# aptx4869lm/4DCapture-FPV

Hardware: AMD Instinct MI355X
Metric: frames/sec global-opt (fixed iters), 1024f clip/500k-pt scene; Chamfer GB/s (higher is better)
Workload: dtype f32; 1 GPU; BASELINE config 3: 1024-frame clip, 500000-pt scene, 500 contact verts, 500 Adam iterations (phase split 0.8), full loss; frames sharded over 1 GPU(s); frames=1024, scene_points=500000, contact_verts=500, iters=500, body_verts=10475, lbs_weights_per_vertex=4

## Files before the change

### 4dcapture-fpv_amd/capi.py

```python
from __future__ import annotations

import ctypes
import os
from ctypes import POINTER, c_char_p, c_double, c_float, c_int32, c_int64, c_void_p

import numpy as np

_HERE = os.path.dirname(os.path.abspath(__file__))
LIB_PATH = os.environ.get("FDCAP_LIB") or os.path.join(_HERE, "libfdcap_hip.so")

NUM_LOSSES = 8
XDIM = 78
PDIM = 75


class FdcapError(RuntimeError):
    pass


class ModelDesc(ctypes.Structure):
    _fields_ = [("num_verts", c_int32), ("v_template", POINTER(c_float)), ("shapedirs", POINTER(c_float)),
                ("num_shape", c_int32), ("posedirs", POINTER(c_float)), ("J_regressor", POINTER(c_float)),
                ("parents", POINTER(c_int32)), ("lbs_weights", POINTER(c_float)),
                ("hands_componentsl", POINTER(c_float)), ("hands_componentsr", POINTER(c_float)),
# ... 26 lines not shown
    "fdcap_ctx_create": (c_int32, [POINTER(ModelDesc), POINTER(c_void_p)]),
    "fdcap_ctx_destroy": (None, [c_void_p]),
    "fdcap_set_scene": (c_int32, [c_void_p, c_void_p, c_int64]),
    "fdcap_debug_scene_hash": (c_int32, [c_void_p, c_void_p]),
    "fdcap_debug_scene_table": (c_int32, [c_void_p, c_int32, c_void_p, POINTER(c_int64)]),
    "fdcap_debug_kernel_forms": (c_int32, [c_void_p, c_int32, c_int32]),
    "fdcap_set_contact_ids": (c_int32, [c_void_p, c_void_p, c_int32]),
    "fdcap_chamfer_fwd": (c_int32, [c_void_p, c_void_p, c_void_p, c_int32, c_int32, c_int32, c_int64, c_void_p,
                                     c_void_p, c_void_p, c_void_p, c_void_p]),
    "fdcap_chamfer_bwd": (c_int32, [c_void_p, c_void_p, c_void_p, c_int32, c_int32, c_int32, c_int64, c_void_p,
                                     c_void_p, c_void_p, c_void_p]),
    "fdcap_chamfer_fwd_scene": (c_int32, [c_void_p, c_void_p, c_int32, c_int32, c_void_p, c_void_p, c_int32, c_void_p]),
    "fdcap_chamfer_bwd_scene": (c_int32, [c_void_p, c_void_p, c_int32, c_int32, c_void_p, c_void_p, c_void_p, c_void_p]),
    "fdcap_set_nn_kernel": (c_int32, [c_int32]),
    "fdcap_vposer_decode": (c_int32, [c_void_p, c_void_p, c_int32, c_int32, c_void_p, c_void_p, c_void_p]),
    "fdcap_vposer_decode_bwd": (c_int32, [c_void_p, c_void_p, c_int32, c_int32, c_void_p, c_void_p, c_void_p, c_void_p]),
    "fdcap_smplx_backward": (c_int32, [c_void_p] * 7 + [c_int32] + [c_void_p] * 9),
    "fdcap_body_forward": (c_int32, [c_void_p, c_void_p, c_int32, c_void_p, c_void_p, c_void_p]),
    "fdcap_world_mesh": (c_int32, [c_void_p, c_void_p, c_int32, c_void_p, c_void_p, c_void_p, c_void_p]),
    "fdcap_params_75_to_78": (c_int32, [c_void_p, c_int32, c_void_p, c_void_p]),
    "fdcap_params_78_to_75": (c_int32, [c_void_p, c_int32, c_void_p, c_void_p]),
    "fdcap_smplx_forward": (c_int32, [c_void_p, c_void_p, c_void_p, c_void_p, c_void_p, c_void_p, c_void_p, c_int32,
                                       c_void_p, c_void_p, c_void_p]),
    "fdcap_opt_create": (c_int32, [c_void_p, POINTER(OptConfig), c_void_p, c_void_p, c_void_p, c_void_p, c_void_p]),
    "fdcap_opt_create_clips": (c_int32, [c_void_p, POINTER(OptConfig), c_int32, c_void_p, c_void_p, c_void_p, c_void_p, c_void_p]),
    "fdcap_opt_set_inputs": (c_int32, [c_void_p, c_void_p, c_void_p, c_void_p, c_void_p, c_void_p]),
    "fdcap_opt_backward": (c_int32, [c_void_p, c_int32, c_int32, c_int32, c_void_p]),
    "fdcap_opt_step": (c_int32, [c_void_p, c_int32, c_int32, c_void_p]),
    "fdcap_opt_backward_and_step": (c_int32, [c_void_p, c_int32, c_int32, c_int32, c_void_p]),
    "fdcap_opt_sync": (c_int32, [c_void_p, c_void_p]),
    "fdcap_opt_run": (c_int32, [c_void_p, c_int32, c_int32, c_int32, c_int32, c_int32, c_void_p, c_int32, c_int32, c_void_p, c_void_p]),
    "fdcap_comm_unique_id": (c_int32, [c_void_p]),
    "fdcap_comm_create": (c_int32, [c_void_p, c_void_p, c_int32, c_int32]),
    "fdcap_comm_destroy": (c_int32, [c_void_p]),
    "fdcap_comm_last_error": (c_char_p, [c_void_p]),
    "fdcap_opt_halo_exchange": (c_int32, [c_void_p, c_void_p]),
    "fdcap_opt_exchange": (c_int32, [c_void_p, c_int32, c_int32, c_void_p]),
    "fdcap_opt_time_exchange": (c_int32, [c_void_p, c_int32, POINTER(c_float), POINTER(c_float), c_void_p]),
    "fdcap_comm_allreduce_f64": (c_int32, [c_void_p, c_void_p, c_int32, c_void_p]),
    "fdcap_opt_state_len": (c_int32, [c_void_p]),
    "fdcap_opt_export_state": (c_int32, [c_void_p, c_void_p, c_void_p]),
    "fdcap_opt_import_state": (c_int32, [c_void_p, c_void_p, c_void_p]),
    "fdcap_opt_check_finite": (c_int32, [c_void_p, c_void_p, c_void_p]),
    "fdcap_opt_set_loss_output": (c_int32, [c_void_p, c_void_p]),
    "fdcap_opt_detect_contact": (c_int32, [c_void_p, c_int32, c_void_p, c_void_p]),
    "fdcap_opt_backward_local2": (c_int32, [c_void_p, c_void_p, c_int32, c_void_p]),
    "fdcap_opt_step_x": (c_int32, [c_void_p, c_int32, c_void_p]),
    "fdcap_opt_set_dct": (c_int32, [c_void_p, c_void_p, c_int32, c_int32, c_void_p, c_void_p]),
    "fdcap_opt_dct_fit": (c_int32, [c_void_p, c_int32, c_int32, c_float, c_void_p, c_int32, c_void_p]),
    "fdcap_opt_backward_dct": (c_int32, [c_void_p, c_float, c_float, c_float, c_int32, c_void_p]),
    "fdcap_opt_set_dct_coef": (c_int32, [c_void_p, c_void_p, c_void_p]),
    "fdcap_opt_get_dct": (c_int32, [c_void_p, c_void_p, c_void_p]),
    "fdcap_opt_get_dct_state": (c_int32, [c_void_p, c_void_p, c_void_p, c_void_p]),
    "fdcap_opt_set_dct_state": (c_int32, [c_void_p, c_void_p, c_void_p, c_void_p]),
    "fdcap_opt_dct_windows": (c_int32, [c_void_p, POINTER(c_int32), POINTER(c_int32)]),
    "fdcap_frame_smoother": (c_int32, [c_void_p, c_void_p, c_int32, c_int32, c_float, c_float, c_float, c_float,
                                        c_void_p, c_int32, c_int32, c_void_p, c_void_p]),
    "fdcap_opt_set_keypoints": (c_int32, [c_void_p, c_void_p, c_void_p]),
    "fdcap_opt_backward_fit2d": (c_int32, [c_void_p, POINTER(Fit2dStage), c_int32, c_void_p]),
    "fdcap_opt_reset_adam": (c_int32, [c_void_p, c_void_p]),
    "fdcap_lbfgs_create": (c_int32, [c_int32, POINTER(LbfgsConfig), POINTER(c_void_p)]),
    "fdcap_lbfgs_destroy": (None, [c_void_p]),
    "fdcap_lbfgs_reset": (c_int32, [c_void_p, c_void_p]),
    "fdcap_lbfgs_advance": (c_int32, [c_void_p, c_void_p, c_int32, c_void_p, c_void_p, c_int32, c_void_p, c_void_p]),
    "fdcap_lbfgs_get_stats": (c_int32, [c_void_p, c_void_p, c_void_p, c_void_p, c_void_p]),
    "fdcap_lbfgs_finalize": (c_int32, [c_void_p, c_void_p, c_int32, c_void_p, c_void_p]),
    "fdcap_opt_fit2d_lbfgs": (c_int32, [c_void_p, POINTER(Fit2dStage), POINTER(LbfgsConfig), c_int32, POINTER(c_int32), c_void_p]),
    "fdcap_opt_fit2d_lbfgs_stats": (c_int32, [c_void_p, c_void_p, c_void_p, c_void_p, c_void_p]),
    "fdcap_opt_step_rows_and_pack": (c_int32, [c_void_p, c_int32, c_int32, c_void_p, c_void_p]),
    "fdcap_opt_unpack_and_step_scale": (c_int32, [c_void_p, c_int32, c_int32, c_void_p, c_int32, c_int32, c_void_p]),
    "fdcap_opt_forward_ahead": (c_int32, [c_void_p, c_int32, c_int32, c_int32, c_void_p]),
    "fdcap_exchange_len": (c_int32, []),
    "fdcap_opt_get_results": (c_int32, [c_void_p, c_void_p, c_void_p, c_void_p, c_void_p]),
    "fdcap_opt_destroy": (None, [c_void_p]),
    "fdcap_opt_forward_world": (c_int32, [c_void_p, c_void_p, c_void_p, c_void_p]),
    "fdcap_opt_get_contact": (c_int32, [c_void_p, c_void_p, c_void_p, c_void_p]),
    "fdcap_opt_get_grads": (c_int32, [c_void_p, c_void_p, c_void_p, c_void_p]),
    "fdcap_panel_gemm": (c_int32, [c_void_p, c_int32, c_int32, c_int32, c_void_p, c_int64, c_int64, c_int32, c_void_p, c_int32,
                                   c_void_p]),
    "fdcap_time_blend_gemm": (c_int32, [c_void_p, c_int32, c_int32, POINTER(c_float), c_void_p]),
    "fdcap_opt_nn_timing": (c_int32, [c_void_p, c_int32]),
    "fdcap_opt_nn_timing_read": (c_int32, [c_void_p, POINTER(c_float), POINTER(c_int32)]),
    "fdcap_debug_nn_query_order": (c_int32, [c_void_p, c_int32, c_void_p, c_int32]),
    "fdcap_opt_launch_timing": (c_int32, [c_void_p, c_int32]),
    "fdcap_opt_launch_timing_read": (c_int32, [c_void_p, c_void_p, c_void_p]),
    "fdcap_opt_time_chamfer": (c_int32, [c_void_p, c_int32, c_int32, POINTER(c_float), c_void_p]),
}

_lib = None


def load_library(path: str | None = None) -> ctypes.CDLL:
    global _lib
    if _lib is not None and path is None:
        return _lib
    p = path or LIB_PATH
    if not os.path.exists(p):
        raise FdcapError(f"{p} is missing: build it with `python -c 'import __graft_entry__ as g; g.build()'` "
                         "(hipcc --offload-arch=gfx950).  There is no CPU fallback.")
    lib = ctypes.CDLL(p)
    for name, (res, args) in SYMBOLS.items():
        fn = getattr(lib, name)
        fn.restype = res
        fn.argtypes = args
    info = lib.fdcap_build_info().decode()
    if "packed_fp32=off" not in info and os.environ.get("FDCAP_ALLOW_PK_F32") != "1":
        raise FdcapError(f"{p} was built with packed fp32 instructions ({info}): results are not reliable next to another kernel's "
                         "MFMAs on the same CU (NOTES.md section 6).  Rebuild with __graft_entry__.build(), or set "
                         "FDCAP_ALLOW_PK_F32=1 for an instrumentation variant.")
    if path is None:
        _lib = lib
    return lib


def count_packed_fp32(path: str | None = None) -> int:
    import re
    import shutil
    import subprocess
    import tempfile
    objdump = os.environ.get("LLVM_OBJDUMP", "/opt/rocm/lib/llvm/bin/llvm-objdump")
    if not os.path.exists(objdump):
        raise FdcapError(f"{objdump} not found (set LLVM_OBJDUMP)")
    with tempfile.TemporaryDirectory() as tmp:
        so = os.path.join(tmp, "lib.so")
        shutil.copy(path or LIB_PATH, so)
        subprocess.run([objdump, "--offloading", so], check=True, capture_output=True, cwd=tmp)
        objs = [f for f in os.listdir(tmp) if "amdgcn" in f]
        if not objs:
            raise FdcapError("no gfx950 code object found in the library")
        n = 0
        for f in objs:
            txt = subprocess.run([objdump, "-d", os.path.join(tmp, f)], check=True, capture_output=True, text=True).stdout
            n += len(re.findall(r"\bv_pk_(?:fma|mul|add)_f32\b", txt))
        return n


def check(code: int, what: str) -> None:
    if code == 0:
        return
    if code < 0:
        names = {-1: "FDCAP_E_ARG", -2: "FDCAP_E_STATE", -3: "FDCAP_E_NODEVICE", -4: "FDCAP_E_COMM (RCCL)"}
        raise FdcapError(f"{what}: {names.get(code, code)}")
    raise FdcapError(f"{what}: hipError_t {code}")


def _f32(a):
    return np.ascontiguousarray(a, dtype=np.float32)


def _fp(a):
    return a.ctypes.data_as(POINTER(c_float))


def dptr(t):
    if t is None:
        return None
    if not t.is_cuda:
        raise FdcapError("expected a device tensor (the HIP path has no host fallback)")
    if not t.is_contiguous():
        raise FdcapError("expected a contiguous tensor")
    return c_void_p(t.data_ptr())


def current_stream():
    import torch
    return c_void_p(torch.cuda.current_stream().cuda_stream)
# ... 57 lines not shown
```

### 4dcapture-fpv_amd/csrc/fdc_api_opt.h

```cpp
#pragma once

extern "C" {

void fdcap_opt_destroy(fdcap_ctx* c) {
    if (!c || !c->opt) return;
    OptState* o = c->opt;
    DevBuf<float>* fb[] = {&o->X0, &o->mask, &o->mX, &o->vX, &o->mCAM, &o->vCAM, &o->mS, &o->vS,
                           &o->H1, &o->H2, &o->O, &o->dO, &o->Opart, &o->dZpart, &o->Rm, &o->PF, &o->Jrest, &o->G, &o->A, &o->M,
                           &o->Jw, &o->Voff, &o->Vw, &o->dist, &o->pd, &o->dVoff, &o->dA, &o->dtransl_v, &o->dMv,
                           &o->dsv, &o->dPF, &o->dJw, &o->dX, &o->dCAM, &o->dscale_row, &o->loss_rows, &o->VoffF, &o->VwF, &o->dVF};
    for (auto* b : fb) b->release();
    o->dctD.release(); o->dctCoef.release(); o->dctM.release(); o->dctV.release(); o->adam_tab.release();
    o->idx.release(); o->pi.release(); o->seedpt.release(); o->kp2d.release(); o->floss.release();
    if (o->lbfgs) { fdcap_lbfgs_destroy(o->lbfgs); o->lbfgs = nullptr; }
    o->nnc_ids.release(); o->nnc_hdr.release(); o->nnc_anchor.release();
    for (hipEvent_t e : o->nn_ev) (void)hipEventDestroy(e);
    o->nn_ev.clear();
    for (hipEvent_t e : o->lt.ev) (void)hipEventDestroy(e);
    o->lt.ev.clear(); o->lt.what.clear(); o->lt.on = false; o->lt.used = 0;
    delete o;
    c->opt = nullptr;
}

static_assert(LROW == FDCAP_NUM_LOSSES, "a batch's per-clip loss slots are LROW apart on the device");
// ... 263 lines not shown

int fdcap_opt_set_loss_output(fdcap_ctx* c, double* losses_d) {
    if (!c || !c->opt || !losses_d) return FDCAP_E_ARG;
    c->opt->log_pending = false;
    c->opt->log_dst = nullptr;
    c->opt->losses.p = losses_d;
    return FDCAP_OK;
}

int fdcap_opt_forward_ahead(fdcap_ctx* c, int32_t ii, int32_t P, int32_t log_terms, void* stream) {
    if (!c || !c->opt || c->opt->nclip > 1) return FDCAP_E_STATE;
    { int es_ = opt_sync(c, (hipStream_t)stream); if (es_) return es_; }
    OptState* o = c->opt;
    hipStream_t st = (hipStream_t)stream;
    const int nl = o->cfg.n_local, nc = c->nc;
    int e = opt_pose_forward(c, 2, 2 + nl, st);
    if (e) return e;
    const bool contact_fwd = o->contact_on && ((ii < P && o->cfg.phase1_contact != 0.f) || log_terms);
    if (contact_fwd) HIP_TRY(blend_forward(c->contact, o->PF.p + 2 * NPFX, nl, o->Voff.p + (size_t)2 * nc * 3, st));
    o->ahead = true;
    o->ahead_blend = contact_fwd;
    return (int)hipGetLastError();
}

int fdcap_opt_backward(fdcap_ctx* c, int32_t ii, int32_t P, int32_t log_terms, void* stream) {
    if (!c || !c->opt) return FDCAP_E_STATE;
    const fdcap_opt_config& cf = c->opt->cfg;
    const bool phase2 = ii >= P;
    LossWeights lw;
    lw.rec = 1.f;
    lw.smooth = phase2 ? cf.phase2_smooth : cf.phase1_smooth;
    lw.contact = phase2 ? 0.f : cf.phase1_contact;
    lw.world = phase2 ? cf.phase2_world : 0.f;
    lw.dct = 0.f;
    lw.world_on = phase2;
    return opt_backward_impl(c, lw, log_terms, (hipStream_t)stream);
}

int fdcap_opt_backward_and_step(fdcap_ctx* c, int32_t ii, int32_t P, int32_t log_terms, void* stream) {
    if (!c || !c->opt) return FDCAP_E_STATE;
    OptState* o = c->opt;
    const fdcap_opt_config& cf = o->cfg;
    const bool fuse = opt_whole_clips(o) && o->dctW == 0;
    if (!fuse) {
        const int e = fdcap_opt_backward(c, ii, P, log_terms, stream);
        return e ? e : fdcap_opt_step(c, ii, P, stream);
    }
    const bool phase2 = ii >= P;
    LossWeights lw;
    lw.rec = 1.f;
    lw.smooth = phase2 ? cf.phase2_smooth : cf.phase1_smooth;
    lw.contact = phase2 ? 0.f : cf.phase1_contact;
    lw.world = phase2 ? cf.phase2_world : 0.f;
    lw.dct = 0.f;
    lw.world_on = phase2;
    return opt_backward_impl(c, lw, log_terms, (hipStream_t)stream, ii, P);
}

int fdcap_debug_nn_query_order(fdcap_ctx* c, int32_t mode, const int32_t* perm_host, int32_t n) {
    if (!c || !c->opt) return FDCAP_E_STATE;
    if (mode < 0 || mode > 2) return FDCAP_E_ARG;
    OptState* o = c->opt;
    NNOrder& ord = o->nn_order;
    if (!o->contact_on || ord.qbuf == nullptr) return FDCAP_E_STATE;
    const int nq = o->cfg.n_local * c->nc;
    if (mode == 2) {
        if (!perm_host || n != nq) return FDCAP_E_ARG;
        std::vector<char> seen((size_t)nq, 0);
        for (int i = 0; i < nq; ++i) {
            if (perm_host[i] < 0 || perm_host[i] >= nq || seen[perm_host[i]]) return FDCAP_E_ARG;
            seen[perm_host[i]] = 1;
        }
    }
    HIP_TRY(hipDeviceSynchronize());
    if (mode == 2) HIP_TRY(hipMemcpy(ord.qbuf, perm_host, (size_t)nq * sizeof(int), hipMemcpyHostToDevice));
    HIP_TRY(hipMemset(o->nnc_hdr.p, 0xFF, (size_t)(nq + 31) / 32 * sizeof(int)));
    ord.perm_mode = mode;
    ord.perm_n = mode == 2 ? nq : 0;
    ord.sorted_groups = 0;
    ord.age = 0;
    return FDCAP_OK;
}

}
```

### 4dcapture-fpv_amd/csrc/fdc_scene.h

```cpp
#pragma once
#include <hip/hip_runtime.h>

#include <algorithm>
#include <utility>
#include <vector>

#include "fdc_chamfer.h"

namespace fdc {

constexpr int SC_RS_ROUNDS = 16;
constexpr int SC_RS_TILE = 256 * SC_RS_ROUNDS;
constexpr int SC_SCAN_BATCH = 16;
constexpr int SC_PT_TILE = 1024;
constexpr int SC_SUPER = 16;

__device__ __forceinline__ unsigned sc_key(float v) {
    unsigned u = __float_as_uint(v);
    if ((u << 1) == 0u) u = 0u;
    return (u & 0x80000000u) ? ~u : (u | 0x80000000u);
}

__global__ __launch_bounds__(256) void sc_keys_kernel(const float* __restrict__ xyz, int n, int axis, unsigned* __restrict__ keys,
                                                      int* __restrict__ vals) {
    const int i = blockIdx.x * 256 + threadIdx.x;
    if (i < n) { keys[i] = sc_key(xyz[3 * (size_t)i + axis]); vals[i] = i; }
}

__global__ __launch_bounds__(256) void sc_rs_hist_kernel(const unsigned* __restrict__ keys, int n, int shift, unsigned* __restrict__ hist, int nb) {
    __shared__ unsigned h[256];
    h[threadIdx.x] = 0;
    __syncthreads();
    const int base = blockIdx.x * SC_RS_TILE;
    for (int r = 0; r < SC_RS_ROUNDS; ++r) {
        const int i = base + r * 256 + threadIdx.x;
        if (i < n) atomicAdd(&h[(keys[i] >> shift) & 255u], 1u);
    }
    __syncthreads();
    hist[(size_t)threadIdx.x * nb + blockIdx.x] = h[threadIdx.x];
}

__global__ __launch_bounds__(1024) void sc_scan_kernel(unsigned* __restrict__ a, int m) {
    __shared__ unsigned part[1024];
    a += (size_t)blockIdx.x * m;
    const int per = (m + 1023) / 1024;
    const int lo = min(m, (int)threadIdx.x * per), hi = min(m, lo + per);
    unsigned s = 0;
    for (int i0 = lo; i0 < hi; i0 += SC_SCAN_BATCH) {
        unsigned v[SC_SCAN_BATCH];
#pragma unroll
        for (int k = 0; k < SC_SCAN_BATCH; ++k) v[k] = i0 + k < hi ? a[i0 + k] : 0u;
#pragma unroll
        for (int k = 0; k < SC_SCAN_BATCH; ++k) s += v[k];
    }
    part[threadIdx.x] = s;
    __syncthreads();
    for (int o = 1; o < 1024; o <<= 1) {
        unsigned t = threadIdx.x >= (unsigned)o ? part[threadIdx.x - o] : 0u;
        __syncthreads();
        part[threadIdx.x] += t;
        __syncthreads();
    }
    unsigned run = part[threadIdx.x] - s;
    for (int i0 = lo; i0 < hi; i0 += SC_SCAN_BATCH) {
        unsigned v[SC_SCAN_BATCH];
#pragma unroll
        for (int k = 0; k < SC_SCAN_BATCH; ++k) v[k] = i0 + k < hi ? a[i0 + k] : 0u;
#pragma unroll
        for (int k = 0; k < SC_SCAN_BATCH; ++k)
            if (i0 + k < hi) { a[i0 + k] = run; run += v[k]; }
    }
}

__global__ __launch_bounds__(256) void sc_rs_scatter_kernel(const unsigned* __restrict__ kin, const int* __restrict__ vin,
                                                            unsigned* __restrict__ kout, int* __restrict__ vout, int n, int shift,
                                                            const unsigned* __restrict__ hist, int nb) {
    __shared__ unsigned base[256];
    __shared__ unsigned wcnt[4][256];
    const int tid = threadIdx.x, wave = tid >> 6, lane = tid & 63;
    base[tid] = hist[(size_t)tid * nb + blockIdx.x];
    const int tile0 = blockIdx.x * SC_RS_TILE;
    for (int r = 0; r < SC_RS_ROUNDS; ++r) {
        const int i = tile0 + r * 256 + tid;
        const bool valid = i < n;
        const unsigned key = valid ? kin[i] : 0u;
        const int val = valid ? vin[i] : 0;
        const unsigned d = (key >> shift) & 255u;
        unsigned long long m = __ballot(valid);
#pragma unroll
        for (int b = 0; b < 8; ++b) {
            const bool bit = (d >> b) & 1u;
            const unsigned long long bal = __ballot(bit);
            m &= bit ? bal : ~bal;
        }
        const int rank = __popcll(m & ((1ull << lane) - 1ull));
        for (int k = 0; k < 4; ++k) wcnt[k][tid] = 0;
        __syncthreads();
        if (valid && rank == 0) wcnt[wave][d] = (unsigned)__popcll(m);
        __syncthreads();
        if (valid) {
            unsigned off = base[d];
            for (int k = 0; k < wave; ++k) off += wcnt[k][d];
            kout[off + rank] = key;
            vout[off + rank] = val;
        }
        __syncthreads();
        base[tid] += wcnt[0][tid] + wcnt[1][tid] + wcnt[2][tid] + wcnt[3][tid];
        __syncthreads();
    }
}

static inline size_t nn_query_order_ints(int nq) { return 4 * (size_t)nq + 256 * (size_t)((nq + SC_RS_TILE - 1) / SC_RS_TILE); }

__global__ __launch_bounds__(256) void nn_order_keys_kernel(const float4* __restrict__ seedpt, int nq, unsigned* __restrict__ key,
                                                            int* __restrict__ val, int* __restrict__ hdr, int groups) {
    const int i = blockIdx.x * 256 + threadIdx.x;
    if (i < nq) {
        const int pos = __float_as_int(seedpt[i].w);
        key[i] = pos >= 0 ? min((unsigned)pos >> 7, 0xFFFFu) : 0xFFFFu;
        val[i] = i;
    }
    if (i < groups) hdr[i] = -1;
}

static inline hipError_t nn_query_order(const float4* seedpt, int nq, int* qbuf, int* hdr, int groups, hipStream_t st) {
    const int nb = (nq + SC_RS_TILE - 1) / SC_RS_TILE;
    int* const perm = qbuf;
    int* const val = qbuf + nq;
    unsigned* const key = (unsigned*)(qbuf + 2 * (size_t)nq);
    unsigned* const hist = key + 2 * (size_t)nq;
    hipLaunchKernelGGL(nn_order_keys_kernel, dim3((std::max(nq, groups) + 255) / 256), dim3(256), 0, st, seedpt, nq, key, perm, hdr, groups);
    for (int pass = 0; pass < 2; ++pass) {
        unsigned* const kin = key + (size_t)pass * nq;
        unsigned* const kout = key + (size_t)(1 - pass) * nq;
        hipLaunchKernelGGL(sc_rs_hist_kernel, dim3(nb), dim3(256), 0, st, kin, nq, 8 * pass, hist, nb);
        hipLaunchKernelGGL(sc_scan_kernel, dim3(1), dim3(1024), 0, st, hist, 256 * nb);
        hipLaunchKernelGGL(sc_rs_scatter_kernel, dim3(nb), dim3(256), 0, st, kin, pass ? val : perm, kout, pass ? perm : val, nq, 8 * pass, hist, nb);
    }
    return hipGetLastError();
}

__device__ __forceinline__ int sc_find_node(const int4* __restrict__ nodes, int nn, int p) {
    int lo = 0, hi = nn - 1;
    while (lo < hi) {
        const int mid = (lo + hi + 1) >> 1;
        if (nodes[mid].x <= p) lo = mid; else hi = mid - 1;
    }
    return lo;
}

__global__ __launch_bounds__(256) void sc_axis_kernel(const int4* __restrict__ nodes, int nn, const float* __restrict__ xyz,
                                                      const int* __restrict__ Lx, const int* __restrict__ Ly, const int* __restrict__ Lz,
                                                      unsigned char* __restrict__ axis) {
    const int i = blockIdx.x * 256 + threadIdx.x;
    if (i >= nn) return;
    const int4 nd = nodes[i];
    int ax = 0;
    if (nd.z < nd.y) {
        const int a = nd.x, b = nd.x + nd.y - 1;
        const float ex = xyz[3 * (size_t)Lx[b]] - xyz[3 * (size_t)Lx[a]];
        const float ey = xyz[3 * (size_t)Ly[b] + 1] - xyz[3 * (size_t)Ly[a] + 1];
        const float ez = xyz[3 * (size_t)Lz[b] + 2] - xyz[3 * (size_t)Lz[a] + 2];
        float best = ex;
        if (ey > best) { ax = 1; best = ey; }
        if (ez > best) { ax = 2; }
    }
    axis[i] = (unsigned char)ax;
}

__global__ __launch_bounds__(256) void sc_side_kernel(const int4* __restrict__ nodes, int nn, const unsigned char* __restrict__ axis,
                                                      const int* __restrict__ Lx, const int* __restrict__ Ly, const int* __restrict__ Lz,
                                                      int n, unsigned char* __restrict__ side) {
    const int p = blockIdx.x * 256 + threadIdx.x;
    if (p >= n) return;
    const int nd = sc_find_node(nodes, nn, p);
    const int4 d = nodes[nd];
    const int ax = axis[nd];
    const int id = (ax == 0 ? Lx : ax == 1 ? Ly : Lz)[p];
    side[id] = (unsigned char)((p - d.x) >= d.z);
}

struct ScLists { const int* in[4]; int* out[4]; };

__device__ __forceinline__ int sc_wave_incl_scan(int v) {
    const int lane = threadIdx.x & 63;
#pragma unroll
    for (int o = 1; o < 64; o <<= 1) { const int t = __shfl_up(v, o); if (lane >= o) v += t; }
    return v;
}

__global__ __launch_bounds__(256) void sc_part_count_kernel(ScLists L, const unsigned char* __restrict__ side, int n, unsigned* __restrict__ cnt, int nb) {
    __shared__ unsigned tot[4];
    if (threadIdx.x < 4) tot[threadIdx.x] = 0;
    __syncthreads();
    const int p0 = blockIdx.x * SC_PT_TILE + threadIdx.x * 4;
    for (int l = 0; l < 4; ++l) {
        int c = 0;
        for (int k = 0; k < 4; ++k) if (p0 + k < n) c += side[L.in[l][p0 + k]];
        const int s = sc_wave_incl_scan(c);
        if ((threadIdx.x & 63) == 63) atomicAdd(&tot[l], (unsigned)s);
    }
    __syncthreads();
    if (threadIdx.x < 4) cnt[(size_t)threadIdx.x * nb + blockIdx.x] = tot[threadIdx.x];
}

__global__ __launch_bounds__(256) void sc_part_scatter_kernel(ScLists L, const unsigned char* __restrict__ side, int n,
                                                              const int4* __restrict__ nodes, int nn, const unsigned* __restrict__ cnt, int nb) {
    __shared__ int wsum[4];
    const int tid = threadIdx.x, wave = tid >> 6;
    const int p0 = blockIdx.x * SC_PT_TILE + tid * 4;
    int4 nd[4];
    for (int k = 0; k < 4; ++k) nd[k] = nodes[sc_find_node(nodes, nn, min(p0 + k, n - 1))];
    for (int l = 0; l < 4; ++l) {
        int id[4], s[4], c = 0;
        for (int k = 0; k < 4; ++k) {
            id[k] = p0 + k < n ? L.in[l][p0 + k] : 0;
            s[k] = p0 + k < n ? side[id[k]] : 0;
            c += s[k];
        }
        const int inc = sc_wave_incl_scan(c);
        __syncthreads();
        if ((tid & 63) == 63) wsum[wave] = inc;
        __syncthreads();
        int ones = (int)cnt[(size_t)l * nb + blockIdx.x] + inc - c;
        for (int k = 0; k < wave; ++k) ones += wsum[k];
        for (int k = 0; k < 4; ++k) {
            const int p = p0 + k;
            if (p < n) {
                const int in_node = ones - nd[k].w;
                const int dst = s[k] ? nd[k].x + nd[k].z + in_node : nd[k].x + (p - nd[k].x - in_node);
                L.out[l][dst] = id[k];
            }
            ones += s[k];
        }
    }
}

__device__ __forceinline__ unsigned sc_bf16(float f) {
    unsigned u = __float_as_uint(f);
    u += 0x7FFFu + ((u >> 16) & 1u);
    return u >> 16;
}
__device__ __forceinline__ float sc_bf16f(unsigned h) { return __uint_as_float(h << 16); }
__device__ __forceinline__ float sc_pad(float lo, float hi) {
#pragma clang fp contract(off)
    return 1e-6f + 1e-6f * fmaxf(fabsf(lo), fabsf(hi));
}

__global__ __launch_bounds__(MF_CH) void sc_finalize_kernel(const float* __restrict__ xyz, const int* __restrict__ order, int n,
                                                            float4* __restrict__ orig, float4* __restrict__ sorted, int* __restrict__ inv,
                                                            float4* __restrict__ bounds, float4* __restrict__ qbounds,
                                                            uint4* __restrict__ frags, float4* __restrict__ centers) {
#pragma clang fp contract(off)
    static_assert(MF_CH % 256 == 0 && MF_CH / 4 % 64 == 0, "a quarter cell is a whole number of waves");
    constexpr int NW = MF_CH / 64, WPQ = NW / 4;
    __shared__ float wlo[NW][3], whi[NW][3], wr2[NW];
    __shared__ float cen[3];
    const int ch = blockIdx.x, j = threadIdx.x, wave = j >> 6, lane = j & 63;
    const int p = ch * MF_CH + j;
    const bool valid = p < n;
    float x = 0.f, y = 0.f, z = 0.f;
    int idx = 0;
    if (valid) {
        idx = order[p];
        x = xyz[3 * (size_t)idx]; y = xyz[3 * (size_t)idx + 1]; z = xyz[3 * (size_t)idx + 2];
        const float4 pt = make_float4(x, y, z, __int_as_float(idx));
        sorted[p] = pt;
        orig[idx] = pt;
        inv[idx] = p;
    }
    float lo[3] = {valid ? x : INFINITY, valid ? y : INFINITY, valid ? z : INFINITY};
    float hi[3] = {valid ? x : -INFINITY, valid ? y : -INFINITY, valid ? z : -INFINITY};
// ... 65 lines not shown
        lo.x = fminf(lo.x, a.x); lo.y = fminf(lo.y, a.y); lo.z = fminf(lo.z, a.z);
        hi.x = fmaxf(hi.x, b.x); hi.y = fmaxf(hi.y, b.y); hi.z = fmaxf(hi.z, b.z);
    }
    sb[2 * (size_t)su] = lo; sb[2 * (size_t)su + 1] = hi;
}

inline void sc_split(int64_t n, int64_t* nleft) {
    const int64_t unit = n > MF_CH ? MF_CH : 32;
    const int64_t units = (n + unit - 1) / unit;
    *nleft = std::min(n - 1, (units / 2) * unit);
}

inline void sc_level_tables(int64_t ns, std::vector<int4>* nodes, std::vector<int>* level_off) {
    nodes->clear(); level_off->clear();
    std::vector<std::pair<int64_t, int64_t>> cur, nxt;
    if (ns > 0) cur.push_back({0, ns});
    for (;;) {
        bool any = false;
        for (auto& nd : cur) any = any || nd.second > 32;
        if (!any) break;
        level_off->push_back((int)nodes->size());
        int64_t ones = 0;
        nxt.clear();
        for (auto& nd : cur) {
            const int64_t a = nd.first, n = nd.second;
            int64_t nl = n;
            if (n > 32) sc_split(n, &nl);
            nodes->push_back(make_int4((int)a, (int)n, (int)nl, (int)ones));
            ones += n - nl;
            if (nl < n) { nxt.push_back({a, nl}); nxt.push_back({a + nl, n - nl}); }
            else nxt.push_back({a, n});
        }
        cur.swap(nxt);
    }
    level_off->push_back((int)nodes->size());
}

inline void scene_order_host(const float* xyz, int64_t ns, std::vector<int>& order) {
    order.resize((size_t)ns);
    for (int64_t i = 0; i < ns; ++i) order[i] = (int)i;
    std::vector<std::pair<int64_t, int64_t>> stack;
    if (ns > 0) stack.push_back({0, ns});
    while (!stack.empty()) {
        const int64_t a = stack.back().first, b = stack.back().second;
        stack.pop_back();
        const int64_t n = b - a;
        if (n <= 32) { std::sort(order.begin() + a, order.begin() + b); continue; }
        int64_t nleft;
        sc_split(n, &nleft);
        float blo[3] = {1e30f, 1e30f, 1e30f}, bhi[3] = {-1e30f, -1e30f, -1e30f};
        for (int64_t p = a; p < b; ++p)
            for (int k = 0; k < 3; ++k) { float v = xyz[3 * (int64_t)order[p] + k]; blo[k] = std::min(blo[k], v); bhi[k] = std::max(bhi[k], v); }
        int ax = 0;
        for (int k = 1; k < 3; ++k) if (bhi[k] - blo[k] > bhi[ax] - blo[ax]) ax = k;
        std::nth_element(order.begin() + a, order.begin() + a + nleft, order.begin() + b, [&](int i, int j) {
            const float vi = xyz[3 * (int64_t)i + ax], vj = xyz[3 * (int64_t)j + ax];
            return vi < vj || (vi == vj && i < j);
        });
        stack.push_back({a, a + nleft});
        stack.push_back({a + nleft, b});
    }
}

struct SceneTables {
    float4* orig; float4* sorted; int* inv; float4* bounds; float4* qbounds; float4* sbounds; uint4* frags; float4* centers;
};

inline hipError_t scene_build_device(const float* xyz_host, int64_t ns64, const SceneTables& T, const int* order_host) {
#define SC_TRY(e) do { hipError_t e_ = (e); if (e_ != hipSuccess) { if (arena) (void)hipFree(arena); return e_; } } while (0)
    char* arena = nullptr;
    const int ns = (int)ns64;
    if (ns <= 0) return hipSuccess;
    const int nchunk = (ns + MF_CH - 1) / MF_CH, nsuper = (nchunk + SC_SUPER - 1) / SC_SUPER;
    const int nb_rs = (ns + SC_RS_TILE - 1) / SC_RS_TILE, nb_pt = (ns + SC_PT_TILE - 1) / SC_PT_TILE;
    std::vector<int4> nodes;
    std::vector<int> level_off;
    if (!order_host) sc_level_tables(ns, &nodes, &level_off);
    const int nlev = order_host ? 0 : (int)level_off.size() - 1;
    int max_nodes = 1;
    for (int l = 0; l < nlev; ++l) max_nodes = std::max(max_nodes, level_off[l + 1] - level_off[l]);
    auto al = [](size_t b) { return (b + 255) & ~(size_t)255; };
    const size_t o_xyz = 0, o_list = o_xyz + al((size_t)ns * 12), o_key = o_list + 8 * al((size_t)ns * 4),
                 o_side = o_key + 2 * al((size_t)ns * 4), o_hist = o_side + al((size_t)ns),
                 o_cnt = o_hist + al((size_t)256 * nb_rs * 4), o_nodes = o_cnt + al((size_t)4 * nb_pt * 4),
                 o_axis = o_nodes + al(std::max<size_t>(nodes.size(), 1) * sizeof(int4)), total = o_axis + al((size_t)max_nodes);
    SC_TRY(hipMalloc((void**)&arena, total));
    float* xyz = (float*)(arena + o_xyz);
    int* list[4][2];
    for (int l = 0; l < 4; ++l) for (int b = 0; b < 2; ++b) list[l][b] = (int*)(arena + o_list + (size_t)(2 * l + b) * al((size_t)ns * 4));
    unsigned* key[2] = {(unsigned*)(arena + o_key), (unsigned*)(arena + o_key + al((size_t)ns * 4))};
    unsigned char* side = (unsigned char*)(arena + o_side);
    unsigned* hist = (unsigned*)(arena + o_hist);
    unsigned* cnt = (unsigned*)(arena + o_cnt);
    int4* d_nodes = (int4*)(arena + o_nodes);
    unsigned char* axis = (unsigned char*)(arena + o_axis);
    hipStream_t st = 0;
    SC_TRY(hipMemcpyAsync(xyz, xyz_host, (size_t)ns * 12, hipMemcpyHostToDevice, st));
    const int* order = nullptr;
    if (order_host) {
        SC_TRY(hipMemcpyAsync(list[3][0], order_host, (size_t)ns * 4, hipMemcpyHostToDevice, st));
        order = list[3][0];
    } else {
        if (!nodes.empty()) SC_TRY(hipMemcpyAsync(d_nodes, nodes.data(), nodes.size() * sizeof(int4), hipMemcpyHostToDevice, st));
        const dim3 g256((ns + 255) / 256);
        for (int ax = 0; ax < 3; ++ax) {
            hipLaunchKernelGGL(sc_keys_kernel, g256, dim3(256), 0, st, xyz, ns, ax, key[0], list[ax][0]);
            for (int pass = 0; pass < 4; ++pass) {
                const int a = pass & 1, b = a ^ 1;
                hipLaunchKernelGGL(sc_rs_hist_kernel, dim3(nb_rs), dim3(256), 0, st, key[a], ns, 8 * pass, hist, nb_rs);
                hipLaunchKernelGGL(sc_scan_kernel, dim3(1), dim3(1024), 0, st, hist, 256 * nb_rs);
                hipLaunchKernelGGL(sc_rs_scatter_kernel, dim3(nb_rs), dim3(256), 0, st, key[a], list[ax][a], key[b], list[ax][b], ns, 8 * pass, hist, nb_rs);
            }
        }
        hipLaunchKernelGGL(sc_keys_kernel, g256, dim3(256), 0, st, xyz, ns, 0, key[0], list[3][0]);
        int cur = 0;
        for (int l = 0; l < nlev; ++l) {
            const int4* nd = d_nodes + level_off[l];
            const int nn = level_off[l + 1] - level_off[l];
            hipLaunchKernelGGL(sc_axis_kernel, dim3((nn + 255) / 256), dim3(256), 0, st, nd, nn, xyz, list[0][cur], list[1][cur], list[2][cur], axis);
            hipLaunchKernelGGL(sc_side_kernel, g256, dim3(256), 0, st, nd, nn, axis, list[0][cur], list[1][cur], list[2][cur], ns, side);
            ScLists L;
            for (int k = 0; k < 4; ++k) { L.in[k] = list[k][cur]; L.out[k] = list[k][cur ^ 1]; }
            hipLaunchKernelGGL(sc_part_count_kernel, dim3(nb_pt), dim3(256), 0, st, L, side, ns, cnt, nb_pt);
            hipLaunchKernelGGL(sc_scan_kernel, dim3(4), dim3(1024), 0, st, cnt, nb_pt);
            hipLaunchKernelGGL(sc_part_scatter_kernel, dim3(nb_pt), dim3(256), 0, st, L, side, ns, nd, nn, cnt, nb_pt);
            cur ^= 1;
        }
        order = list[3][cur];
    }
    hipLaunchKernelGGL(sc_finalize_kernel, dim3(nchunk), dim3(MF_CH), 0, st, xyz, order, ns, T.orig, T.sorted, T.inv, T.bounds, T.qbounds,
                       T.frags, T.centers);
    hipLaunchKernelGGL(sc_super_kernel, dim3((nsuper + 255) / 256), dim3(256), 0, st, T.bounds, nchunk, T.sbounds, nsuper);
    SC_TRY(hipGetLastError());
    SC_TRY(hipStreamSynchronize(st));
    (void)hipFree(arena);
    return hipSuccess;
#undef SC_TRY
}

}
```

### include/fdcap.h

```cpp
#ifndef FDCAP_H
#define FDCAP_H

#include <stdint.h>

#ifdef __cplusplus
extern "C" {
#endif

#define FDCAP_OK 0
#define FDCAP_E_ARG (-1)
#define FDCAP_E_STATE (-2)
#define FDCAP_E_NODEVICE (-3)
#define FDCAP_E_COMM (-4)
#define FDCAP_UNIQUE_ID_BYTES 128

#define FDCAP_NUM_JOINTS 55
#define FDCAP_XDIM 78
#define FDCAP_PDIM 75
#define FDCAP_MAX_SCENE_POINTS 67000000
#define FDCAP_NUM_LOSSES 8

typedef struct fdcap_ctx fdcap_ctx;

typedef struct fdcap_model_desc {
// ... 94 lines not shown
int fdcap_opt_run(fdcap_ctx* ctx, int32_t ii0, int32_t ii1, int32_t num_iter, int32_t first_phase2_iter, int32_t log_every,
                  double* hist_d, int32_t hist_rows, int32_t flags, int32_t* n_logged, void* stream);
int32_t fdcap_opt_state_len(fdcap_ctx* ctx);
int fdcap_opt_export_state(fdcap_ctx* ctx, float* state_d, void* stream);
int fdcap_opt_import_state(fdcap_ctx* ctx, const float* state_d, void* stream);
int fdcap_opt_check_finite(fdcap_ctx* ctx, int32_t* count_d, void* stream);
int fdcap_opt_set_loss_output(fdcap_ctx* ctx, double* losses_d);
int fdcap_opt_detect_contact(fdcap_ctx* ctx, int32_t n_left, float* weight_left_d, void* stream);
int fdcap_opt_backward_local2(fdcap_ctx* ctx, const float* contact_weight_d, int32_t n_left, void* stream);
int fdcap_opt_step_x(fdcap_ctx* ctx, int32_t step, void* stream);

int fdcap_opt_set_dct(fdcap_ctx* ctx, const float* dct_mtx, int32_t T, int32_t C, const float* c_dct_d, void* stream);
int fdcap_opt_dct_fit(fdcap_ctx* ctx, int32_t iters, int32_t step0, float weight, float* obj_hist_d,
                      int32_t log_stride, void* stream);
int fdcap_opt_backward_dct(fdcap_ctx* ctx, float w_dct, float w_rec, float w_contact, int32_t log_terms, void* stream);
int fdcap_opt_set_dct_coef(fdcap_ctx* ctx, const float* c_dct_d, void* stream);
int fdcap_opt_get_dct(fdcap_ctx* ctx, float* c_dct_d, void* stream);
int fdcap_opt_get_dct_state(fdcap_ctx* ctx, float* m_d, float* v_d, void* stream);
int fdcap_opt_set_dct_state(fdcap_ctx* ctx, const float* m_d, const float* v_d, void* stream);
int32_t fdcap_opt_dct_windows(fdcap_ctx* ctx, int32_t* w0, int32_t* w1);

int fdcap_frame_smoother(fdcap_ctx* ctx, const float* data78_d, int32_t N, int32_t iters, float lr, float w_rec,
                         float w_vposer, float w_prev, float* state_d, int32_t step0, int32_t has_prev,
                         float* out78_d, void* stream);

typedef struct fdcap_fit2d_stage {
    float fx, fy, cx, cy;
    float rho;
    float w_data, w_pose, w_shape, w_hand;
} fdcap_fit2d_stage;
int fdcap_opt_set_keypoints(fdcap_ctx* ctx, const float* kp_d, void* stream);
int fdcap_opt_backward_fit2d(fdcap_ctx* ctx, const fdcap_fit2d_stage* stage, int32_t log_terms, void* stream);
int fdcap_opt_reset_adam(fdcap_ctx* ctx, void* stream);

typedef struct fdcap_lbfgs_config {
    int32_t dim, history, max_iter, max_eval, max_steps, max_ls;
    float lr, tolerance_grad, tolerance_change, ftol, gtol;
} fdcap_lbfgs_config;
typedef struct fdcap_lbfgs fdcap_lbfgs;
int fdcap_lbfgs_create(int32_t n_problems, const fdcap_lbfgs_config* cfg, fdcap_lbfgs** out);
void fdcap_lbfgs_destroy(fdcap_lbfgs* opt);
int fdcap_lbfgs_reset(fdcap_lbfgs* opt, void* stream);
int fdcap_lbfgs_advance(fdcap_lbfgs* opt, float* x_d, int32_t x_stride, const float* f_d, const float* g_d, int32_t g_stride,
                        int32_t* n_active_d, void* stream);
int fdcap_lbfgs_finalize(fdcap_lbfgs* opt, float* x_d, int32_t x_stride, int32_t* n_unfinished_d, void* stream);
int fdcap_lbfgs_get_stats(fdcap_lbfgs* opt, int32_t* iterations_d, int32_t* evaluations_d, float* loss_d, void* stream);

int fdcap_opt_fit2d_lbfgs(fdcap_ctx* ctx, const fdcap_fit2d_stage* stage, const fdcap_lbfgs_config* cfg, int32_t max_rounds,
                          int32_t* rounds_out, void* stream);
int fdcap_opt_fit2d_lbfgs_stats(fdcap_ctx* ctx, int32_t* iterations_d, int32_t* evaluations_d, float* loss_d, void* stream);

int fdcap_opt_step_rows_and_pack(fdcap_ctx* ctx, int32_t ii, int32_t first_phase2_iter, float* send_d, void* stream);
int fdcap_opt_unpack_and_step_scale(fdcap_ctx* ctx, int32_t ii, int32_t first_phase2_iter, const float* gathered_d,
                                    int32_t rank, int32_t world, void* stream);
int32_t fdcap_exchange_len(void);

int fdcap_comm_unique_id(uint8_t* id128);
int fdcap_comm_create(fdcap_ctx* ctx, const uint8_t* id128, int32_t rank, int32_t world);
int fdcap_comm_destroy(fdcap_ctx* ctx);
const char* fdcap_comm_last_error(fdcap_ctx* ctx);
int fdcap_opt_halo_exchange(fdcap_ctx* ctx, void* stream);
int fdcap_opt_exchange(fdcap_ctx* ctx, int32_t ii, int32_t first_phase2_iter, void* stream);
int fdcap_opt_time_exchange(fdcap_ctx* ctx, int32_t iters, float* us_exchange, float* us_allgather, void* stream);
int fdcap_comm_allreduce_f64(fdcap_ctx* ctx, double* buf_d, int32_t n, void* stream);
int fdcap_opt_forward_ahead(fdcap_ctx* ctx, int32_t ii, int32_t first_phase2_iter, int32_t log_terms, void* stream);

int fdcap_opt_get_results(fdcap_ctx* ctx, float* body_rec75_d, float* scale_d, float* cam_ext_d,
                          void* stream);
void fdcap_opt_destroy(fdcap_ctx* ctx);

int fdcap_opt_forward_world(fdcap_ctx* ctx, float* verts_d, float* joints_d, void* stream);
int fdcap_opt_get_contact(fdcap_ctx* ctx, float* dist_d, int32_t* idx_d, void* stream);
int fdcap_opt_get_grads(fdcap_ctx* ctx, float* dx_d, float* dcam_d, void* stream);

int fdcap_time_blend_gemm(fdcap_ctx* ctx, int32_t rows, int32_t iters, float* ms, void* stream);

int fdcap_panel_gemm(const float* A_d, int32_t lda, int32_t M, int32_t K, const float* B_h, int64_t sk, int64_t sn, int32_t N,
                     float* C_d, int32_t ldc, void* stream);

int fdcap_opt_nn_timing(fdcap_ctx* ctx, int32_t max_launches);
int fdcap_opt_nn_timing_read(fdcap_ctx* ctx, float* mean_ms, int32_t* launches);

int fdcap_debug_nn_query_order(fdcap_ctx* ctx, int32_t mode, const int32_t* perm_h, int32_t n);

#define FDCAP_LT_VPOSER_FWD 0
#define FDCAP_LT_POSE_FWD 1
#define FDCAP_LT_CONTACT_FWD 2
#define FDCAP_LT_CHAMFER_NN 3
#define FDCAP_LT_SKIN_BWD 4
#define FDCAP_LT_BLEND_BWD 5
#define FDCAP_LT_POSE_BWD 6
#define FDCAP_LT_VPOSER_BWD 7
#define FDCAP_LT_NUM 8
int fdcap_opt_launch_timing(fdcap_ctx* ctx, int32_t max_events);
int fdcap_opt_launch_timing_read(fdcap_ctx* ctx, float* mean_us , int32_t* counts );

int fdcap_opt_time_chamfer(fdcap_ctx* ctx, int32_t iters, int32_t brute_force, float* ms, void* stream);

#ifdef __cplusplus
}
#endif
#endif
```

Measured before the change: 17220 frames/s.

## Parallelize radix-sort scan across digits and fuse key generation into sort passes

```diff
diff --git a/4dcapture-fpv_amd/capi.py b/4dcapture-fpv_amd/capi.py
--- a/4dcapture-fpv_amd/capi.py
+++ b/4dcapture-fpv_amd/capi.py
@@ -132,6 +132,8 @@
     "fdcap_opt_nn_timing": (c_int32, [c_void_p, c_int32]),
     "fdcap_opt_nn_timing_read": (c_int32, [c_void_p, POINTER(c_float), POINTER(c_int32)]),
     "fdcap_debug_nn_query_order": (c_int32, [c_void_p, c_int32, c_void_p, c_int32]),
+    "fdcap_debug_nn_query_perm": (c_int32, [c_void_p, c_void_p, c_int32]),
+    "fdcap_debug_query_order_of": (c_int32, [c_void_p, c_int32, c_void_p]),
     "fdcap_opt_launch_timing": (c_int32, [c_void_p, c_int32]),
     "fdcap_opt_launch_timing_read": (c_int32, [c_void_p, c_void_p, c_void_p]),
     "fdcap_opt_time_chamfer": (c_int32, [c_void_p, c_int32, c_int32, POINTER(c_float), c_void_p]),
diff --git a/4dcapture-fpv_amd/csrc/fdc_api_opt.h b/4dcapture-fpv_amd/csrc/fdc_api_opt.h
--- a/4dcapture-fpv_amd/csrc/fdc_api_opt.h
+++ b/4dcapture-fpv_amd/csrc/fdc_api_opt.h
@@ -369,4 +369,34 @@
     return FDCAP_OK;
 }
 
-}
+int fdcap_debug_nn_query_perm(fdcap_ctx* c, int32_t* perm_out_host, int32_t n) {
+    if (!c || !c->opt) return FDCAP_E_STATE;
+    OptState* o = c->opt;
+    const NNOrder& ord = o->nn_order;
+    const int nq = o->cfg.n_local * c->nc;
+    if (!o->contact_on || ord.qbuf == nullptr || ord.perm_n != nq || nq <= 0) return FDCAP_E_STATE;
+    if (!perm_out_host || n != nq) return FDCAP_E_ARG;
+    HIP_TRY(hipDeviceSynchronize());
+    HIP_TRY(hipMemcpy(perm_out_host, ord.qbuf, (size_t)nq * sizeof(int), hipMemcpyDeviceToHost));
+    return FDCAP_OK;
+}
+
+int fdcap_debug_query_order_of(const int32_t* pos_host, int32_t n, int32_t* perm_out_host) {
+    if (!pos_host || !perm_out_host || n <= 0) return FDCAP_E_ARG;
+    std::vector<float4> sp((size_t)n);
+    for (int i = 0; i < n; ++i) { sp[i] = make_float4(0.f, 0.f, 0.f, 0.f); memcpy(&sp[i].w, &pos_host[i], 4); }
+    const int groups = (n + 31) / 32;
+    DevBuf<float4> seedpt;
+    DevBuf<int> qbuf, hdr;
+    hipError_t e = seedpt.ensure((size_t)n);
+    if (e == hipSuccess) e = qbuf.ensure(nn_query_order_ints(n));
+    if (e == hipSuccess) e = hdr.ensure((size_t)groups);
+    if (e == hipSuccess) e = hipMemcpy(seedpt.p, sp.data(), (size_t)n * sizeof(float4), hipMemcpyHostToDevice);
+    if (e == hipSuccess) e = nn_query_order(seedpt.p, n, qbuf.p, hdr.p, groups, (hipStream_t)0);
+    if (e == hipSuccess) e = hipStreamSynchronize((hipStream_t)0);
+    if (e == hipSuccess) e = hipMemcpy(perm_out_host, qbuf.p, (size_t)n * sizeof(int), hipMemcpyDeviceToHost);
+    seedpt.release(); qbuf.release(); hdr.release();
+    return e == hipSuccess ? FDCAP_OK : (int)e;
+}
+
+}
diff --git a/4dcapture-fpv_amd/csrc/fdc_scene.h b/4dcapture-fpv_amd/csrc/fdc_scene.h
--- a/4dcapture-fpv_amd/csrc/fdc_scene.h
+++ b/4dcapture-fpv_amd/csrc/fdc_scene.h
@@ -11,7 +11,6 @@
 
 constexpr int SC_RS_ROUNDS = 16;
 constexpr int SC_RS_TILE = 256 * SC_RS_ROUNDS;
-constexpr int SC_SCAN_BATCH = 16;
 constexpr int SC_PT_TILE = 1024;
 constexpr int SC_SUPER = 16;
 
@@ -27,81 +26,104 @@
     if (i < n) { keys[i] = sc_key(xyz[3 * (size_t)i + axis]); vals[i] = i; }
 }
 
-__global__ __launch_bounds__(256) void sc_rs_hist_kernel(const unsigned* __restrict__ keys, int n, int shift, unsigned* __restrict__ hist, int nb) {
+__device__ __forceinline__ int sc_wave_incl_scan(int v) {
+    const int lane = threadIdx.x & 63;
+#pragma unroll
+    for (int o = 1; o < 64; o <<= 1) { const int t = __shfl_up(v, o); if (lane >= o) v += t; }
+    return v;
+}
+
+struct ScKeyArray {
+    const unsigned* __restrict__ keys;
+    __device__ __forceinline__ unsigned operator()(int i) const { return keys[i]; }
+};
+struct NnQuarterKey {
+    const float4* __restrict__ seedpt;
+    __device__ __forceinline__ unsigned operator()(int i) const {
+        const int pos = __float_as_int(seedpt[i].w);
+        return pos >= 0 ? min((unsigned)pos >> 7, 0xFFFFu) : 0xFFFFu;
+    }
+};
+
+template <class Key>
+__global__ __launch_bounds__(256) void sc_rs_hist_kernel(Key keyof, int n, int shift, unsigned* __restrict__ hist, int nb,
+                                                         int* __restrict__ hdr, int groups) {
     __shared__ unsigned h[256];
     h[threadIdx.x] = 0;
     __syncthreads();
     const int base = blockIdx.x * SC_RS_TILE;
     for (int r = 0; r < SC_RS_ROUNDS; ++r) {
         const int i = base + r * 256 + threadIdx.x;
-        if (i < n) atomicAdd(&h[(keys[i] >> shift) & 255u], 1u);
-    }
+        if (i < n) atomicAdd(&h[(keyof(i) >> shift) & 255u], 1u);
+    }
+    for (int g = blockIdx.x * 256 + threadIdx.x; g < groups; g += gridDim.x * 256) hdr[g] = -1;
     __syncthreads();
     hist[(size_t)threadIdx.x * nb + blockIdx.x] = h[threadIdx.x];
 }
 
-__global__ __launch_bounds__(1024) void sc_scan_kernel(unsigned* __restrict__ a, int m) {
-    __shared__ unsigned part[1024];
+__global__ __launch_bounds__(1024) void sc_scan_kernel(unsigned* __restrict__ a, int m, unsigned* __restrict__ tot) {
+    __shared__ unsigned wsum[2][16];
     a += (size_t)blockIdx.x * m;
-    const int per = (m + 1023) / 1024;
-    const int lo = min(m, (int)threadIdx.x * per), hi = min(m, lo + per);
-    unsigned s = 0;
-    for (int i0 = lo; i0 < hi; i0 += SC_SCAN_BATCH) {
-        unsigned v[SC_SCAN_BATCH];
+    const int tid = threadIdx.x, wave = tid >> 6;
+    unsigned carry = 0;
+    for (int c0 = 0, par = 0; c0 < m; c0 += 1024, par ^= 1) {
+        const int i = c0 + tid;
+        const unsigned v = i < m ? a[i] : 0u;
+        const unsigned inc = (unsigned)sc_wave_incl_scan((int)v);
+        if ((tid & 63) == 63) wsum[par][wave] = inc;
+        __syncthreads();
+        unsigned before = carry;
+        for (int k = 0; k < 16; ++k) { const unsigned t = wsum[par][k]; carry += t; if (k < wave) before += t; }
+        if (i < m) a[i] = before + inc - v;
+    }
+    if (tid == 0 && tot) tot[blockIdx.x] = carry;
+}
+
+__device__ __forceinline__ int sc_wave_match(unsigned d, bool valid, int* count) {
+    unsigned long long m = __ballot(valid);
 #pragma unroll
-        for (int k = 0; k < SC_SCAN_BATCH; ++k) v[k] = i0 + k < hi ? a[i0 + k] : 0u;
-#pragma unroll
-        for (int k = 0; k < SC_SCAN_BATCH; ++k) s += v[k];
-    }
-    part[threadIdx.x] = s;
-    __syncthreads();
-    for (int o = 1; o < 1024; o <<= 1) {
-        unsigned t = threadIdx.x >= (unsigned)o ? part[threadIdx.x - o] : 0u;
-        __syncthreads();
-        part[threadIdx.x] += t;
-        __syncthreads();
-    }
-    unsigned run = part[threadIdx.x] - s;
-    for (int i0 = lo; i0 < hi; i0 += SC_SCAN_BATCH) {
-        unsigned v[SC_SCAN_BATCH];
-#pragma unroll
-        for (int k = 0; k < SC_SCAN_BATCH; ++k) v[k] = i0 + k < hi ? a[i0 + k] : 0u;
-#pragma unroll
-        for (int k = 0; k < SC_SCAN_BATCH; ++k)
-            if (i0 + k < hi) { a[i0 + k] = run; run += v[k]; }
-    }
-}
-
-__global__ __launch_bounds__(256) void sc_rs_scatter_kernel(const unsigned* __restrict__ kin, const int* __restrict__ vin,
-                                                            unsigned* __restrict__ kout, int* __restrict__ vout, int n, int shift,
-                                                            const unsigned* __restrict__ hist, int nb) {
+    for (int b = 0; b < 8; ++b) {
+        const bool bit = (d >> b) & 1u;
+        const unsigned long long bal = __ballot(bit);
+        m &= bit ? bal : ~bal;
+    }
+    *count = __popcll(m);
+    return __popcll(m & ((1ull << (threadIdx.x & 63)) - 1ull));
+}
+
+template <class Key>
+__global__ __launch_bounds__(256) void sc_rs_scatter_kernel(Key keyof, const int* __restrict__ vin, unsigned* __restrict__ kout,
+                                                            int* __restrict__ vout, int n, int shift, const unsigned* __restrict__ hist,
+                                                            const unsigned* __restrict__ tot, int nb) {
     __shared__ unsigned base[256];
     __shared__ unsigned wcnt[4][256];
+    __shared__ unsigned wtot[4];
     const int tid = threadIdx.x, wave = tid >> 6, lane = tid & 63;
-    base[tid] = hist[(size_t)tid * nb + blockIdx.x];
+    const unsigned t = tot[tid];
+    const unsigned inc = (unsigned)sc_wave_incl_scan((int)t);
+    if (lane == 63) wtot[wave] = inc;
+    for (int k = 0; k < 4; ++k) wcnt[k][tid] = 0;
+    __syncthreads();
+    unsigned digit_base = inc - t + hist[(size_t)tid * nb + blockIdx.x];
+    for (int k = 0; k < wave; ++k) digit_base += wtot[k];
+    base[tid] = digit_base;
     const int tile0 = blockIdx.x * SC_RS_TILE;
     for (int r = 0; r < SC_RS_ROUNDS; ++r) {
         const int i = tile0 + r * 256 + tid;
         const bool valid = i < n;
-        const unsigned key = valid ? kin[i] : 0u;
-        const int val = valid ? vin[i] : 0;
+        const unsigned key = valid ? keyof(i) : 0u;
+        const int val = valid ? (vin ? vin[i] : i) : 0;
         const unsigned d = (key >> shift) & 255u;
-        unsigned long long m = __ballot(valid);
-#pragma unroll
-        for (int b = 0; b < 8; ++b) {
-            const bool bit = (d >> b) & 1u;
-            const unsigned long long bal = __ballot(bit);
-            m &= bit ? bal : ~bal;
-        }
-        const int rank = __popcll(m & ((1ull << lane) - 1ull));
-        for (int k = 0; k < 4; ++k) wcnt[k][tid] = 0;
-        __syncthreads();
-        if (valid && rank == 0) wcnt[wave][d] = (unsigned)__popcll(m);
+        int cnt;
+        const int rank = sc_wave_match(d, valid, &cnt);
+        if (r) for (int k = 0; k < 4; ++k) wcnt[k][tid] = 0;
+        __syncthreads();
+        if (valid && rank == 0) wcnt[wave][d] = (unsigned)cnt;
         __syncthreads();
         if (valid) {
             unsigned off = base[d];
             for (int k = 0; k < wave; ++k) off += wcnt[k][d];
-            kout[off + rank] = key;
+            if (kout) kout[off + rank] = key;
             vout[off + rank] = val;
         }
         __syncthreads();
@@ -110,33 +132,26 @@
     }
 }
 
-static inline size_t nn_query_order_ints(int nq) { return 4 * (size_t)nq + 256 * (size_t)((nq + SC_RS_TILE - 1) / SC_RS_TILE); }
-
-__global__ __launch_bounds__(256) void nn_order_keys_kernel(const float4* __restrict__ seedpt, int nq, unsigned* __restrict__ key,
-                                                            int* __restrict__ val, int* __restrict__ hdr, int groups) {
-    const int i = blockIdx.x * 256 + threadIdx.x;
-    if (i < nq) {
-        const int pos = __float_as_int(seedpt[i].w);
-        key[i] = pos >= 0 ? min((unsigned)pos >> 7, 0xFFFFu) : 0xFFFFu;
-        val[i] = i;
-    }
-    if (i < groups) hdr[i] = -1;
-}
+template <class Key>
+static inline void sc_rs_pass(Key keyof, const int* vin, unsigned* kout, int* vout, int n, int shift, unsigned* hist, unsigned* tot,
+                              int* hdr, int groups, hipStream_t st) {
+    const int nb = (n + SC_RS_TILE - 1) / SC_RS_TILE;
+    hipLaunchKernelGGL(sc_rs_hist_kernel<Key>, dim3(nb), dim3(256), 0, st, keyof, n, shift, hist, nb, hdr, groups);
+    hipLaunchKernelGGL(sc_scan_kernel, dim3(256), dim3(1024), 0, st, hist, nb, tot);
+    hipLaunchKernelGGL(sc_rs_scatter_kernel<Key>, dim3(nb), dim3(256), 0, st, keyof, vin, kout, vout, n, shift, hist, tot, nb);
+}
+
+static inline size_t nn_query_order_ints(int nq) { return 3 * (size_t)nq + 256 * (size_t)((nq + SC_RS_TILE - 1) / SC_RS_TILE) + 256; }
 
 static inline hipError_t nn_query_order(const float4* seedpt, int nq, int* qbuf, int* hdr, int groups, hipStream_t st) {
     const int nb = (nq + SC_RS_TILE - 1) / SC_RS_TILE;
     int* const perm = qbuf;
     int* const val = qbuf + nq;
     unsigned* const key = (unsigned*)(qbuf + 2 * (size_t)nq);
-    unsigned* const hist = key + 2 * (size_t)nq;
-    hipLaunchKernelGGL(nn_order_keys_kernel, dim3((std::max(nq, groups) + 255) / 256), dim3(256), 0, st, seedpt, nq, key, perm, hdr, groups);
-    for (int pass = 0; pass < 2; ++pass) {
-        unsigned* const kin = key + (size_t)pass * nq;
-        unsigned* const kout = key + (size_t)(1 - pass) * nq;
-        hipLaunchKernelGGL(sc_rs_hist_kernel, dim3(nb), dim3(256), 0, st, kin, nq, 8 * pass, hist, nb);
-        hipLaunchKernelGGL(sc_scan_kernel, dim3(1), dim3(1024), 0, st, hist, 256 * nb);
-        hipLaunchKernelGGL(sc_rs_scatter_kernel, dim3(nb), dim3(256), 0, st, kin, pass ? val : perm, kout, pass ? perm : val, nq, 8 * pass, hist, nb);
-    }
+    unsigned* const hist = key + nq;
+    unsigned* const tot = hist + 256 * (size_t)nb;
+    sc_rs_pass(NnQuarterKey{seedpt}, nullptr, key, val, nq, 0, hist, tot, hdr, groups, st);
+    sc_rs_pass(ScKeyArray{key}, val, nullptr, perm, nq, 8, hist, tot, nullptr, 0, st);
     return hipGetLastError();
 }
 
@@ -181,13 +196,6 @@
 }
 
 struct ScLists { const int* in[4]; int* out[4]; };
-
-__device__ __forceinline__ int sc_wave_incl_scan(int v) {
-    const int lane = threadIdx.x & 63;
-#pragma unroll
-    for (int o = 1; o < 64; o <<= 1) { const int t = __shfl_up(v, o); if (lane >= o) v += t; }
-    return v;
-}
 
 __global__ __launch_bounds__(256) void sc_part_count_kernel(ScLists L, const unsigned char* __restrict__ side, int n, unsigned* __restrict__ cnt, int nb) {
     __shared__ unsigned tot[4];
@@ -419,7 +427,7 @@
     auto al = [](size_t b) { return (b + 255) & ~(size_t)255; };
     const size_t o_xyz = 0, o_list = o_xyz + al((size_t)ns * 12), o_key = o_list + 8 * al((size_t)ns * 4),
                  o_side = o_key + 2 * al((size_t)ns * 4), o_hist = o_side + al((size_t)ns),
-                 o_cnt = o_hist + al((size_t)256 * nb_rs * 4), o_nodes = o_cnt + al((size_t)4 * nb_pt * 4),
+                 o_cnt = o_hist + al((size_t)256 * (nb_rs + 1) * 4), o_nodes = o_cnt + al((size_t)4 * nb_pt * 4),
                  o_axis = o_nodes + al(std::max<size_t>(nodes.size(), 1) * sizeof(int4)), total = o_axis + al((size_t)max_nodes);
     SC_TRY(hipMalloc((void**)&arena, total));
     float* xyz = (float*)(arena + o_xyz);
@@ -428,6 +436,7 @@
     unsigned* key[2] = {(unsigned*)(arena + o_key), (unsigned*)(arena + o_key + al((size_t)ns * 4))};
     unsigned char* side = (unsigned char*)(arena + o_side);
     unsigned* hist = (unsigned*)(arena + o_hist);
+    unsigned* tot = hist + (size_t)256 * nb_rs;
     unsigned* cnt = (unsigned*)(arena + o_cnt);
     int4* d_nodes = (int4*)(arena + o_nodes);
     unsigned char* axis = (unsigned char*)(arena + o_axis);
@@ -444,9 +453,7 @@
             hipLaunchKernelGGL(sc_keys_kernel, g256, dim3(256), 0, st, xyz, ns, ax, key[0], list[ax][0]);
             for (int pass = 0; pass < 4; ++pass) {
                 const int a = pass & 1, b = a ^ 1;
-                hipLaunchKernelGGL(sc_rs_hist_kernel, dim3(nb_rs), dim3(256), 0, st, key[a], ns, 8 * pass, hist, nb_rs);
-                hipLaunchKernelGGL(sc_scan_kernel, dim3(1), dim3(1024), 0, st, hist, 256 * nb_rs);
-                hipLaunchKernelGGL(sc_rs_scatter_kernel, dim3(nb_rs), dim3(256), 0, st, key[a], list[ax][a], key[b], list[ax][b], ns, 8 * pass, hist, nb_rs);
+                sc_rs_pass(ScKeyArray{key[a]}, list[ax][a], pass < 3 ? key[b] : nullptr, list[ax][b], ns, 8 * pass, hist, tot, nullptr, 0, st);
             }
         }
         hipLaunchKernelGGL(sc_keys_kernel, g256, dim3(256), 0, st, xyz, ns, 0, key[0], list[3][0]);
@@ -459,7 +466,7 @@
             ScLists L;
             for (int k = 0; k < 4; ++k) { L.in[k] = list[k][cur]; L.out[k] = list[k][cur ^ 1]; }
             hipLaunchKernelGGL(sc_part_count_kernel, dim3(nb_pt), dim3(256), 0, st, L, side, ns, cnt, nb_pt);
-            hipLaunchKernelGGL(sc_scan_kernel, dim3(4), dim3(1024), 0, st, cnt, nb_pt);
+            hipLaunchKernelGGL(sc_scan_kernel, dim3(4), dim3(1024), 0, st, cnt, nb_pt, (unsigned*)nullptr);
             hipLaunchKernelGGL(sc_part_scatter_kernel, dim3(nb_pt), dim3(256), 0, st, L, side, ns, nd, nn, cnt, nb_pt);
             cur ^= 1;
         }
diff --git a/include/fdcap.h b/include/fdcap.h
--- a/include/fdcap.h
+++ b/include/fdcap.h
@@ -200,6 +200,8 @@
 int fdcap_opt_nn_timing_read(fdcap_ctx* ctx, float* mean_ms, int32_t* launches);
 
 int fdcap_debug_nn_query_order(fdcap_ctx* ctx, int32_t mode, const int32_t* perm_h, int32_t n);
+int fdcap_debug_nn_query_perm(fdcap_ctx* ctx, int32_t* perm_out_h, int32_t n);
+int fdcap_debug_query_order_of(const int32_t* pos_h, int32_t n, int32_t* perm_out_h);
 
 #define FDCAP_LT_VPOSER_FWD 0
 #define FDCAP_LT_POSE_FWD 1
```

New measurement: 17650 frames/s (median of 6 runs). 2.5% higher.
